# lrm2017/Fastest_Image_Pattern_Matching

Hardware: AMD Instinct MI355X
Metric: template matches/sec + ms/search, 4024×3036 src ±180°; HBM GB/s vs roofline (higher is better)
Workload: dtype u8

## Files before the change

### fastest_image_pattern_matching_amd/_lib.py

```python
from __future__ import annotations

import ctypes as C
import os
import subprocess

_HERE = os.path.dirname(os.path.abspath(__file__))
LIB_PATH = os.path.join(_HERE, "lib", "libfpm_hip.so")
CSRC = os.path.join(_HERE, "csrc")

FPM_OK = 0
FPM_E_INVALID_ARG = -1
FPM_E_NOT_LEARNED = -2
FPM_E_SIZE = -3
FPM_E_DEVICE = -4
FPM_E_CAPACITY = -5
FPM_E_INTERNAL = -6

(FMT_GRAY8, FMT_BGR8, FMT_RGB8, FMT_BGRA8, FMT_RGBA8, FMT_BGR8_PLANAR, FMT_RGB8_PLANAR) = range(7)
FMT_COUNT = 7

(K_PYR, K_TOP_WARP, K_TOP_NCC, K_TOP_NMS, K_CAND_INIT, K_ROI_TABLES, K_ROI_WARP, K_ROI_CORR, K_ROI_EVAL, K_ROI_SMALL,
 K_CAND_STEP, K_TOP_MAP, K_NOT, K_PATCH, K_COMPARE, K_LEARN) = range(16)
KERNEL_NAMES = ["pyr_down", "top_warp", "top_ncc", "top_nms", "cand_init", "roi_tables", "roi_warp", "roi_corr",
                "roi_eval", "roi_small", "cand_step", "top_map", "bitwise_not", "patch_warp", "patch_compare"]
# ... 138 lines not shown
    _fields_ = [("x", C.c_int32), ("y", C.c_int32), ("score", C.c_float)]


PEAKS_STATS_CALL, PEAKS_STATS_JOB = 8, 4
PEAKS_RAN_BLOCKS, PEAKS_RAN_NMS, PEAKS_RAN_FAST, PEAKS_RAN_GREEDY = 1, 2, 4, 8
TOP_MAPS_STATS = 8
TOP_FUSED_STATS = 10
TOP_FORM_EXACT16, TOP_FORM_EXACT14, TOP_FORM_SMALL, TOP_FORM_LARGE = 0, 1, 2, 3

_P = C.c_void_p
_U8P = C.POINTER(C.c_uint8)
SIGNATURES = {
    "fpm_params_default": (None, [C.POINTER(Params)]),
    "fpm_abi_version": (C.c_int, []),
    "fpm_create": (C.c_int, [C.c_int, C.POINTER(_P)]),
    "fpm_destroy": (C.c_int, [_P]),
    "fpm_last_error": (C.c_char_p, [_P]),
    "fpm_set_params": (C.c_int, [_P, C.POINTER(Params)]),
    "fpm_get_params": (C.c_int, [_P, C.POINTER(Params)]),
    "fpm_learn": (C.c_int, [_P, _U8P, C.c_int32, C.c_int32, C.c_size_t]),
    "fpm_clear_pattern": (C.c_int, [_P]),
    "fpm_is_learned": (C.c_int, [_P]),
    "fpm_match": (C.c_int, [_P, _U8P, C.c_int32, C.c_int32, C.c_size_t, C.POINTER(Result), C.c_int32,
                            C.POINTER(C.c_int32), C.POINTER(C.c_double)]),
    "fpm_stage_sources": (C.c_int, [_P, C.POINTER(_U8P), C.c_int32, C.c_int32, C.c_int32, C.c_size_t]),
    "fpm_stage_sources_device": (C.c_int, [_P, C.POINTER(_P), C.c_int32, C.c_int32, C.c_int32, C.c_size_t, C.c_size_t,
                                           C.c_int32, _P]),
    "fpm_match_device": (C.c_int, [_P, _P, C.c_int32, C.c_int32, C.c_size_t, C.c_size_t, C.c_int32, _P,
                                   C.POINTER(Result), C.c_int32, C.POINTER(C.c_int32), C.POINTER(C.c_double)]),
    "fpm_match_staged": (C.c_int, [_P, C.POINTER(Result), C.c_int32, C.POINTER(C.c_int32)]),
    "fpm_match_staged_launch": (C.c_int, [_P]),
    "fpm_match_staged_finish": (C.c_int, [_P, C.POINTER(Result), C.c_int32, C.POINTER(C.c_int32)]),
    "fpm_op_pyr_down": (C.c_int, [_P, _U8P, C.c_int32, C.c_int32, C.c_size_t, _U8P, C.c_size_t]),
    "fpm_op_pyr_down2": (C.c_int, [_P, _U8P, C.c_int32, C.c_int32, C.c_size_t, _U8P, C.c_size_t, _U8P, C.c_size_t,
                                   C.c_int32, C.c_int32]),
    "fpm_op_bitwise_not": (C.c_int, [_P, _U8P, C.c_int32, C.c_int32, C.c_size_t, _U8P, C.c_size_t]),
    "fpm_op_to_gray": (C.c_int, [_P, _P, C.c_int32, C.c_int32, C.c_size_t, C.c_size_t, C.c_int32, C.c_int32, _U8P,
                                 C.c_size_t]),
    "fpm_op_warp_affine": (C.c_int, [_P, _U8P, C.c_int32, C.c_int32, C.c_size_t, C.POINTER(C.c_double), _U8P,
                                     C.c_int32, C.c_int32, C.c_size_t, C.c_int32]),
    "fpm_op_ncc_map": (C.c_int, [_P, _U8P, C.c_int32, C.c_int32, C.c_size_t, C.c_int32, C.c_int32,
                                 C.POINTER(C.c_float)]),
    "fpm_op_refine": (C.c_int, [_P, C.POINTER(_U8P), C.c_int32, C.c_int32, C.c_int32, C.c_size_t, C.c_int32,
                                C.POINTER(C.c_float), C.POINTER(C.c_double), C.c_int32, C.c_int32, C.c_int32, C.c_int32,
                                C.POINTER(RoiRecord), _U8P, C.POINTER(C.c_int32)]),
    "fpm_op_peaks": (C.c_int, [_P, C.POINTER(C.POINTER(C.c_float)), C.POINTER(C.c_int32), C.POINTER(C.c_int32),
                               C.c_int32, C.c_int32, C.c_int32, C.c_int32, C.c_int32, C.c_int32, C.c_double, C.c_double,
                               C.c_int32, C.c_int32, C.c_uint32, C.POINTER(Peak), C.POINTER(C.c_int32),
                               C.POINTER(C.c_int32)]),
    "fpm_op_top_maps": (C.c_int, [_P, C.c_int32, C.c_double, C.POINTER(C.c_int32), C.POINTER(C.c_int32),
                                  C.POINTER(C.c_int64), C.POINTER(C.c_int32), C.POINTER(C.c_int32), C.c_int32,
                                  C.POINTER(C.c_float), C.c_int64, C.POINTER(C.c_int32), C.POINTER(C.c_int32),
                                  C.POINTER(C.c_float), C.c_int64, C.POINTER(C.c_int32)]),
    "fpm_op_top_fused": (C.c_int, [_P, C.POINTER(C.c_int32), C.POINTER(C.c_int32), C.POINTER(C.c_int64),
                                   C.POINTER(C.c_int32), C.POINTER(C.c_int32), C.c_int32, C.POINTER(C.c_float),
                                   C.c_int64, C.POINTER(Peak), C.POINTER(C.c_int32), C.POINTER(Peak),
                                   C.POINTER(C.c_int32), C.c_int64, C.POINTER(C.c_int32)]),
    "fpm_op_overlap_filter": (C.c_int, [_P, C.POINTER(C.c_float), C.POINTER(C.c_double), C.c_int32, C.c_double,
                                        C.c_int32, C.POINTER(C.c_int32), C.POINTER(C.c_int32), C.POINTER(C.c_int32)]),
    "fpm_template_info": (C.c_int, [_P, C.POINTER(C.c_int32), C.POINTER(C.c_int32)]),
    "fpm_template_level": (C.c_int, [_P, C.c_int32, C.POINTER(C.c_int32), C.POINTER(C.c_int32),
                                     C.POINTER(C.c_double), C.POINTER(C.c_double), C.POINTER(C.c_double),
                                     C.POINTER(C.c_int32), _U8P, C.c_size_t]),
    "fpm_set_angle_shard": (C.c_int, [_P, C.c_int32, C.c_int32]),
    "fpm_get_angle_shard": (C.c_int, [_P, C.POINTER(C.c_int32), C.POINTER(C.c_int32)]),
    "fpm_last_candidates": (C.c_int, [_P, C.c_int32, C.POINTER(Candidate), C.c_int32, C.POINTER(C.c_int32)]),
# ... 130 lines not shown
```

### fastest_image_pattern_matching_amd/csrc/fpm_engine.hip

```cpp
#include <hip/hip_runtime.h>

#include <algorithm>
#include <array>
#include <cfloat>
#include <chrono>
#include <cmath>
#include <cstddef>
#include <cstdio>
#include <cstdlib>
#include <cstring>
#include <new>
#include <random>
#include <string>
#include <vector>

#include "../../include/fpm.h"
#include "fpm_host.h"
#include "fpm_kernels.h"
#include "fpm_model.h"

using namespace fpm;

namespace {

// ... 3734 lines not shown
    if (!ctx->learned) return FPM_E_NOT_LEARNED;
    if (level < 0 || level >= (int)ctx->tmpl.size()) return FPM_E_INVALID_ARG;
    const TmplLevel& t = ctx->tmpl[level];
    *w = t.w; *h = t.h; *mean = t.mean; *norm = t.norm; *inv_area = t.inv_area; *result_equal1 = t.equal1 ? 1 : 0;
    if (pixels && t.px.empty()) {
        std::vector<uint8_t> px((size_t)t.w * t.h);
        if (hipSetDevice(ctx->device) != hipSuccess ||
            hipMemcpy2D(px.data(), t.w, ctx->d_tmpl.as<uint8_t>() + t.off, t.pitch, t.w, t.h, hipMemcpyDeviceToHost) != hipSuccess)
            return FPM_E_DEVICE;
        t.px = std::move(px);
    }
    if (pixels)
        for (int y = 0; y < t.h; ++y) std::memcpy(pixels + (size_t)y * stride, t.px.data() + (size_t)y * t.w, (size_t)t.w);
    return FPM_OK;
}

int fpm_op_pyr_down(fpm_ctx* ctx, const uint8_t* src, int32_t w, int32_t h, size_t ss, uint8_t* dst, size_t ds) {
    if (!ctx) return FPM_E_INVALID_ARG;
    if (!src || !dst || w <= 0 || h <= 0 || ss < (size_t)w) { ctx->err = "bad image"; return FPM_E_INVALID_ARG; }
    const int dw = (w + 1) / 2, dh = (h + 1) / 2;
    if (ds < (size_t)dw) { ctx->err = "bad dst stride"; return FPM_E_INVALID_ARG; }
    HIP_TRY(hipSetDevice(ctx->device));
    const int sp = round_up(w + 4, 64), dp = round_up(dw + 4, 64);
    HIP_TRY(ctx->d_op_a.ensure((size_t)sp * (h + 1)));
    HIP_TRY(ctx->d_op_b.ensure((size_t)dp * (dh + 1)));
    HIP_TRY(hipMemcpy2DAsync(ctx->d_op_a.p, sp, src, ss, w, h, hipMemcpyHostToDevice, ctx->stream));
    launch_pyr_down(ctx->d_op_a.as<uint8_t>(), w, h, sp, 0, ctx->d_op_b.as<uint8_t>(), dw, dh, dp, 0, 1, ctx->stream, 3);
    HIP_TRY(hipGetLastError());
    HIP_TRY(hipMemcpy2DAsync(dst, ds, ctx->d_op_b.p, dp, dw, dh, hipMemcpyDeviceToHost, ctx->stream));
    HIP_TRY(hipStreamSynchronize(ctx->stream));
    return FPM_OK;
}

int fpm_op_bitwise_not(fpm_ctx* ctx, const uint8_t* src, int32_t w, int32_t h, size_t ss, uint8_t* dst, size_t ds) {
    if (!ctx) return FPM_E_INVALID_ARG;
    if (!src || !dst || w <= 0 || h <= 0 || ss < (size_t)w) { ctx->err = "bad image"; return FPM_E_INVALID_ARG; }
    if (ds < (size_t)w) { ctx->err = "bad dst stride"; return FPM_E_INVALID_ARG; }
    HIP_TRY(hipSetDevice(ctx->device));
    const SrcLevel lv = level_layout(w, h);
    HIP_TRY(ctx->d_op_a.ensure(lv.img_bytes));
    HIP_TRY(hipMemcpy2DAsync(ctx->d_op_a.p, lv.pitch, src, ss, w, h, hipMemcpyHostToDevice, ctx->stream));
    {
        ProfScope ps(ctx, FPM_K_NOT, 2 * (int64_t)w * h);
        if (!launch_bitwise_not(ctx->d_op_a.as<uint8_t>(), w, h, lv.pitch, lv.img_bytes, 1, ctx->stream)) {
            ctx->err = "level layout: rows not 16-byte aligned";
            return FPM_E_INTERNAL;
        }
    }
    HIP_TRY(hipGetLastError());
    HIP_TRY(hipMemcpy2DAsync(dst, ds, ctx->d_op_a.p, lv.pitch, w, h, hipMemcpyDeviceToHost, ctx->stream));
    HIP_TRY(hipStreamSynchronize(ctx->stream));
    prof_collect(ctx);
    return FPM_OK;
}

int fpm_op_to_gray(fpm_ctx* ctx, const void* src, int32_t w, int32_t h, size_t ss, size_t plane_stride, int32_t format,
                   int32_t invert, uint8_t* dst, size_t ds) {
    if (!ctx) return FPM_E_INVALID_ARG;
    if (!src || !dst) { ctx->err = "bad image"; return FPM_E_INVALID_ARG; }
    const int rc = check_image_desc(ctx, 1, w, h, ss, plane_stride, format);
    if (rc != FPM_OK) return rc;
    if (ds < (size_t)w) { ctx->err = "bad dst stride"; return FPM_E_INVALID_ARG; }
    HIP_TRY(hipSetDevice(ctx->device));
    const size_t extent = image_extent(w, h, ss, plane_stride, format);
    const size_t mis = (uintptr_t)src & 15;
    const SrcLevel lv = level_layout(w, h);
// ... 640 lines not shown
```

### fastest_image_pattern_matching_amd/csrc/fpm_kernels.h

```cpp
#pragma once
#include <hip/hip_runtime.h>
#include <stdint.h>

#include "fpm_geom.h"

namespace fpm {

struct WarpJob {
    const uint8_t* src;
    uint8_t* dst;
    int32_t sw, sh, sp;
    int32_t dw, dh, dp;
    int32_t border;
    int32_t pad;
    double M[6];
};

struct NccJob {
    const uint8_t* img;
    const uint8_t* tmpl;
    float* out;
    int32_t iw, ih, ip;
    int32_t tw, th, tp;
    int32_t ow, oh;
// ... 100 lines not shown
    int32_t step;
    int32_t mark_reached0;
    int32_t* live_out;
    int32_t* live_out_count;
    double thr;
    const RoiRecord* prev_rec;
    const AngleNode* prev_nodes;
    double prev_thr;
    int32_t prev_W, prev_H;
    CandState* state_out;
    int32_t* nt_tab;
    const AngleNode* nt_nodes;
    int32_t nt_tabw, nt_tabh, nt_tw, nt_th, nt_W, nt_H;
    uint64_t* stamps;
};


struct PackArgs {
    const int32_t* counts; int32_t J;
    const Peak* peaks; int32_t C;
    int32_t cap;
    const int32_t* livecnt; int32_t nlive;
    const int32_t* live0;
    const int32_t* live0_count;
    const CandState* state;
    const RoiRecord* rec;
    int32_t n3;
    char* host;
    size_t o_counts, o_peaks, o_live, o_live0, o_state0, o_rec0;
};

void launch_pyr_down(const uint8_t* src, int sw, int sh, int sp, size_t s_img, uint8_t* dst, int dw, int dh,
                     int dp, size_t d_img, int nimg, hipStream_t st, int seg_chunks = 0, int32_t* zero = nullptr,
                     int nzero = 0);
void launch_pyr_down2(const uint8_t* src, int sw, int sh, int sp, size_t s_img, uint8_t* bdst, int bw, int bh, int bp,
                      size_t b_img, uint8_t* cdst, int cw, int ch, int cp, size_t c_img, int nimg, hipStream_t st,
                      int seg_chunks = 0, int32_t* zero = nullptr, int nzero = 0, int chunk_rows = 0);
bool launch_bitwise_not(uint8_t* img, int w, int h, int pitch, size_t img_bytes, int nimg, hipStream_t st);
bool launch_stage_gray(const uint8_t* const* d_imgs, int nimg, int w, int h, size_t stride, size_t plane_stride,
                       int format, bool aligned, uint8_t* dst, int pitch, size_t img_bytes, bool invert,
                       hipStream_t st);
int stage_gray_bpp(int format);
void launch_warp(const WarpJob* jobs, int njobs, int max_pixels, hipStream_t st, int32_t* zero = nullptr,
                 int nzero = 0);
struct PatchJob {
    double M[6];
    int64_t out_off;
    int32_t src;
    int32_t pad;
};
struct PatchArgs {
    const PatchJob* jobs;
    int32_t njobs;
    const uint8_t* level0;
    size_t img_stride;
    int32_t sw, sh, sp;
    uint8_t* out;
    size_t row_stride;
    int32_t pw, ph;
    int32_t dword;
    int32_t tiles_x, tiles_y;
};
bool launch_patch_warp(PatchArgs a, hipStream_t st);
enum { kCmpSumI, kCmpSumII, kCmpSumT, kCmpSumTT, kCmpSumIT, kCmpSumAbs, kCmpNOver, kCmpMaxAbs, kCmpX0, kCmpY0, kCmpX1,
       kCmpY1, kCompareFields };
struct CompareAcc {
    uint64_t s[6];
// ... 234 lines not shown
```

### fastest_image_pattern_matching_amd/csrc/fpm_kernels.hip

```cpp
#include <float.h>
#include <stdio.h>
#include <stdlib.h>
#include <limits.h>

#include <map>
#include <mutex>
#include <type_traits>
#include <utility>

#include "../../include/fpm.h"
#include "fpm_kernels.h"
#include "fpm_model.h"
#include "fpm_rrect.h"

static void ensure_lds_attr(const void* fn, size_t bytes) {
    if (bytes <= 65536) return;
    int dev = 0;
    (void)hipGetDevice(&dev);
    static std::mutex mu;
    static std::map<std::pair<int, const void*>, size_t> done;
    std::lock_guard<std::mutex> lock(mu);
    size_t& cur = done[std::make_pair(dev, fn)];
    if (bytes <= cur) return;
    (void)hipFuncSetAttribute(fn, hipFuncAttributeMaxDynamicSharedMemorySize, (int)bytes);
// ... 164 lines not shown
        const uint32_t h2 = __builtin_amdgcn_udot4(PD_K, __builtin_amdgcn_alignbyte(w2, w1, 2), 0, false) + ((w2 >> 16) & 0xff);
        const uint32_t h3 = __builtin_amdgcn_udot4(PD_K, w2, 0, false) + (w3 & 0xff);
        uint2 o;
        o.x = h0 | (h1 << 16);
        o.y = h2 | (h3 << 16);
        *(uint2*)&hs[r][4 * g] = o;
    }
    __syncthreads();
    if (ABL == 3) { if (hs[tid & 63][tid >> 1] == 0x5a5a && tid == 999) dst[0] = 1; return; }
#pragma unroll
    for (int k = 0; k < PD_OH * (PD_OW / 4) / 256; ++k) {
        const int i = tid + 256 * k;
        const int orow = i / (PD_OW / 4), g = i - orow * (PD_OW / 4);
        const int oy = oy0 + orow, ox = ox0 + 4 * g;
        if (oy >= dh || ox >= dw) continue;
        uint32_t acc[4] = {128, 128, 128, 128};
        const int kw[5] = {1, 4, 6, 4, 1};
#pragma unroll
        for (int t = 0; t < 5; ++t) {
            const uint2 q = *(const uint2*)&hs[2 * orow + t][4 * g];
            acc[0] += kw[t] * (q.x & 0xffff); acc[1] += kw[t] * (q.x >> 16);
            acc[2] += kw[t] * (q.y & 0xffff); acc[3] += kw[t] * (q.y >> 16);
        }
        uint8_t* d = dst + (size_t)oy * dp + ox;
        if (ox + 4 <= dw) {
            *(uint32_t*)d = (acc[0] >> 8) | ((acc[1] >> 8) << 8) | ((acc[2] >> 8) << 16) | ((acc[3] >> 8) << 24);
        } else {
            for (int j = 0; j < dw - ox; ++j) d[j] = (uint8_t)(acc[j] >> 8);
        }
    }
}

typedef unsigned short fpm_u16x2 __attribute__((ext_vector_type(2)));

template <int OH>
__global__ __launch_bounds__(256) void k_pyr_down_s(const uint8_t* __restrict__ src0, int sw, int sh, int sp,
                                                    size_t s_img, uint8_t* __restrict__ dst0, int dw, int dh,
                                                    int dp, size_t d_img, int nimg, int32_t* zero, int nzero) {
    constexpr int IH = 2 * OH + 4;
    constexpr int PS_NL = (IH * (PD_IW / 16) + 255) / 256;
    __shared__ __attribute__((aligned(16))) uint8_t tin[IH][PD_IW];
    if (blockIdx.x == 0)
        for (int i = threadIdx.x; i < nzero; i += 256) zero[i] = 0;
    __shared__ __attribute__((aligned(16))) uint16_t hs[IH][PD_OW];
    const int gx = (dw + PD_OW - 1) / PD_OW, chunks = (dh + OH - 1) / OH;
    const long U = (long)gx * chunks * nimg;
    const int w = xcd_remap(blockIdx.x, gridDim.x);
    long u = U * w / gridDim.x;
    const long u_end = U * (w + 1) / gridDim.x;
    const int tid = threadIdx.x;
    while (u < u_end) {
        const long strip = u / chunks;
        const int c0 = (int)(u - strip * chunks);
        const int run = (int)min(u_end - u, (long)(chunks - c0));
        u += run;
        const int bx = (int)(strip % gx), bz = (int)(strip / gx);
        const uint8_t* src = src0 + (size_t)bz * s_img;
        uint8_t* dst = dst0 + (size_t)bz * d_img;
        const int ox0 = bx * PD_OW;
        const int oy_begin = c0 * OH, oy_end = min(dh, (c0 + run) * OH);
        __syncthreads();
        const int ix0 = 2 * ox0 - 16;
        constexpr int Q = PD_IW / 16;
        auto srow = [&](int y) {
            y = y < 0 ? -y : y;
            y = y >= sh ? 2 * sh - 2 - y : y;
            return y < 0 ? 0 : (y >= sh ? sh - 1 : y);
        };
        uint4 v[PS_NL];
        auto issue = [&](int iy, int nrows) {
#pragma unroll
            for (int k = 0; k < PS_NL; ++k) {
                const int i = tid + 256 * k;
                const int r = i / Q, c = i - r * Q;
                const int x = ix0 + 16 * c;
                v[k] = make_uint4(0, 0, 0, 0);
                if (r < nrows && x >= 0 && x + 16 <= sp) v[k] = *(const uint4*)(src + (size_t)srow(iy + r) * sp + x);
            }
        };
        auto commit = [&](int roff, int nrows) {
#pragma unroll
            for (int k = 0; k < PS_NL; ++k) {
                const int i = tid + 256 * k;
                const int r = i / Q, c = i - r * Q;
                if (r < nrows) *(uint4*)&tin[roff + r][16 * c] = v[k];
            }
        };
        const int xlo = 2 * ox0 - 2, xhi = min(2 * (ox0 + PD_OW - 1) + 2, 2 * (dw - 1) + 2);
        const bool edge = xlo < 0 || xhi >= sw;
        issue(2 * oy_begin - 2, IH);
        for (int oyc = oy_begin; oyc < oy_end; oyc += OH) {
            const bool first = oyc == oy_begin;
            const int roff = first ? 0 : 4, nrows = first ? IH : 2 * OH;
            const int iy = 2 * oyc - 2 + roff;
            commit(roff, nrows);
            if (edge) {
                __syncthreads();
                for (int i = tid; i < nrows * 4; i += 256) {
                    const int r = i >> 2, k = i & 3;
                    const int x = k < 2 ? xlo + k : xhi - (k - 2);
                    if ((x < 0 && k < 2) || (x >= sw && k >= 2))
                        tin[roff + r][x - ix0] = src[(size_t)srow(iy + r) * sp + reflect101(x, sw)];
                }
            }
            __syncthreads();
            if (oyc + OH < oy_end) issue(2 * oyc + 2 * OH + 2, 2 * OH);
            const int nh = nrows * (PD_OW / 4);
            for (int i = tid; i < nh; i += 256) {
                const int r = roff + i / (PD_OW / 4), g = i % (PD_OW / 4);
                const uint32_t* w = (const uint32_t*)&tin[r][8 * g + 12];
                const uint32_t w0 = w[0], w1 = w[1], w2 = w[2], w3 = w[3];
                const uint32_t h0 = __builtin_amdgcn_udot4(PD_K, __builtin_amdgcn_alignbyte(w1, w0, 2), (w1 >> 16) & 0xff, false);
                const uint32_t h1 = __builtin_amdgcn_udot4(PD_K, w1, w2 & 0xff, false);
                const uint32_t h2 = __builtin_amdgcn_udot4(PD_K, __builtin_amdgcn_alignbyte(w2, w1, 2), (w2 >> 16) & 0xff, false);
                const uint32_t h3 = __builtin_amdgcn_udot4(PD_K, w2, w3 & 0xff, false);
                uint2 o;
                o.x = h0 | (h1 << 16);
                o.y = h2 | (h3 << 16);
                *(uint2*)&hs[r][4 * g] = o;
            }
            __syncthreads();
#pragma unroll
            for (int k = 0; k < OH * (PD_OW / 4) / 256; ++k) {
                const int i = tid + 256 * k;
                const int orow = i / (PD_OW / 4), g = i - orow * (PD_OW / 4);
                const int oy = oyc + orow, ox = ox0 + 4 * g;
                if (oy >= oy_end || ox >= dw) continue;
                fpm_u16x2 a01 = {128, 128}, a23 = {128, 128};
                constexpr unsigned short kw[5] = {1, 4, 6, 4, 1};
#pragma unroll
                for (int tt = 0; tt < 5; ++tt) {
                    const uint2 q = *(const uint2*)&hs[2 * orow + tt][4 * g];
                    a01 += __builtin_bit_cast(fpm_u16x2, q.x) * kw[tt];
                    a23 += __builtin_bit_cast(fpm_u16x2, q.y) * kw[tt];
                }
                const uint32_t packed = __builtin_amdgcn_perm(__builtin_bit_cast(uint32_t, a23),
                                                              __builtin_bit_cast(uint32_t, a01), 0x07050301u);
                uint8_t* d = dst + (size_t)oy * dp + ox;
                if (ox + 4 <= dw) {
                    *(uint32_t*)d = packed;
                } else {
                    for (int j = 0; j < dw - ox; ++j) d[j] = (uint8_t)(packed >> (8 * j));
                }
            }
            __syncthreads();
            ((uint32_t*)hs[tid >> 6])[tid & 63] = ((uint32_t*)hs[2 * OH + (tid >> 6)])[tid & 63];
            __syncthreads();
        }
    }
}

static const int kPyrWGs = [] {
    const char* e = getenv("FPM_PYR_WGS");
    return e && atoi(e) > 0 ? atoi(e) : 4096;
}();
static const int kPyrOH = [] {
    const char* e = getenv("FPM_PYR_OH");
    return e && atoi(e) == 16 ? 16 : 32;
}();
void launch_pyr_down(const uint8_t* src, int sw, int sh, int sp, size_t s_img, uint8_t* dst, int dw, int dh,
                     int dp, size_t d_img, int nimg, hipStream_t st, int seg_chunks, int32_t* zero, int nzero) {
    if (dw <= 0 || dh <= 0 || nimg <= 0) return;
    const int oh = kPyrOH;
    const int gx = (dw + PD_OW - 1) / PD_OW, chunks = (dh + oh - 1) / oh;
    const long units = (long)gx * chunks * nimg;
    const long g = seg_chunks > 0 ? (units + seg_chunks - 1) / seg_chunks : std::min(units, (long)kPyrWGs);
    if (oh == 16)
        hipLaunchKernelGGL(k_pyr_down_s<16>, dim3((unsigned)g), dim3(256), 0, st, src, sw, sh, sp, s_img, dst, dw, dh,
                           dp, d_img, nimg, zero, nzero);
    else
        hipLaunchKernelGGL(k_pyr_down_s<32>, dim3((unsigned)g), dim3(256), 0, st, src, sw, sh, sp, s_img, dst, dw, dh,
                           dp, d_img, nimg, zero, nzero);
}

constexpr int PD2_OWC = 64;
constexpr int PD2_OWB = 2 * PD2_OWC + 8;
constexpr int PD2_GB = PD2_OWB / 4;
constexpr int PD2_BP = 136;
template <int PD2_OHB>
__global__ __launch_bounds__(256) void k_pyr_down2(const uint8_t* __restrict__ src0, int sw, int sh, int sp,
                                                   size_t s_img, uint8_t* __restrict__ b0, int bw, int bh, int bpp,
                                                   size_t b_img, uint8_t* __restrict__ c0, int cw, int ch, int cpp,
                                                   size_t c_img, int nimg, int32_t* zero, int nzero) {
    constexpr int PD2_IH = 2 * (PD2_OHB + 4) + 4, PD2_RING = PD2_OHB + 6;
    __shared__ __attribute__((aligned(16))) uint8_t tin[PD2_IH][PD_IW];
    __shared__ __attribute__((aligned(16))) uint16_t hs[PD2_IH][PD2_BP];
    __shared__ __attribute__((aligned(16))) uint8_t ring[PD2_RING][PD2_BP];
    __shared__ __attribute__((aligned(16))) uint16_t hc[PD2_RING][PD2_OWC];
    if (blockIdx.x == 0)
        for (int i = threadIdx.x; i < nzero; i += 256) zero[i] = 0;
    const int gx = (cw + PD2_OWC - 1) / PD2_OWC, chunks = (bh + PD2_OHB - 1) / PD2_OHB;
    const long U = (long)gx * chunks * nimg;
    const int w = xcd_remap(blockIdx.x, gridDim.x);
    long u = U * w / gridDim.x;
    const long u_end = U * (w + 1) / gridDim.x;
    const int tid = threadIdx.x;
    constexpr int Q = PD_IW / 16;
    constexpr int NL = (PD2_IH * Q + 255) / 256;
    constexpr unsigned short kw[5] = {1, 4, 6, 4, 1};
    auto srow = [&](int y) {
        y = y < 0 ? -y : y;
        y = y >= sh ? 2 * sh - 2 - y : y;
        return y < 0 ? 0 : (y >= sh ? sh - 1 : y);
    };
    while (u < u_end) {
// ... 5380 lines not shown
```

### fastest_image_pattern_matching_amd/matcher.py

```python
from __future__ import annotations

import ctypes as C
import os
from dataclasses import dataclass
from typing import List, Sequence, Tuple

import numpy as np

from . import _lib as L


@dataclass
class SingleTargetMatch:

    ptLT: Tuple[float, float]
    ptRT: Tuple[float, float]
    ptRB: Tuple[float, float]
    ptLB: Tuple[float, float]
    ptCenter: Tuple[float, float]
    dMatchedAngle: float
    dMatchScore: float

    @staticmethod
    def from_c(r: "L.Result") -> "SingleTargetMatch":
# ... 1204 lines not shown
                                             edges.ctypes.data_as(C.POINTER(L.Edge)),
                                             prof.ctypes.data_as(C.POINTER(C.c_int32)) if profiles else None, stride,
                                             n.value, C.byref(n))
            if rc != L.FPM_OK:
                self._patch_fail(rc, "last_calipers")
        return (summary, edges, prof) if profiles else (summary, edges)

    def calipers_at(self, src_index, lts, angles, cals, cap: int = 8, profiles: bool = False):
        idx, lt, ang = patch_poses(src_index, lts, angles)
        arr = _calipers(cals)
        summary, edges, prof, stride = self._caliper_buffers(len(idx), arr, cap, profiles)
        rc = self._lib.fpm_calipers_at(self._ctx, idx.ctypes.data_as(C.POINTER(C.c_int32)),
                                       lt.ctypes.data_as(C.POINTER(C.c_float)), ang.ctypes.data_as(C.POINTER(C.c_double)),
                                       len(idx), arr.ctypes.data_as(C.POINTER(L.Caliper)), len(arr), int(cap),
                                       summary.ctypes.data_as(C.POINTER(L.CaliperSummary)),
                                       edges.ctypes.data_as(C.POINTER(L.Edge)),
                                       prof.ctypes.data_as(C.POINTER(C.c_int32)) if profiles else None, stride)
        if rc != L.FPM_OK:
            self._patch_fail(rc, "calipers_at")
        return (summary, edges, prof) if profiles else (summary, edges)

    def caliper_profile(self):
        ms, n, b = C.c_double(), C.c_int64(), C.c_int64()
        if self._lib.fpm_caliper_profile(self._ctx, C.byref(ms), C.byref(n), C.byref(b)) != L.FPM_OK:
            raise ValueError("fpm_caliper_profile failed")
        return ms.value, n.value, b.value

    def pyr_down(self, img) -> np.ndarray:
        g = _gray(img)
        h, w = g.shape
        out = np.zeros(((h + 1) // 2, (w + 1) // 2), np.uint8)
        rc = self._check(self._lib.fpm_op_pyr_down(self._ctx, L.u8ptr(g), w, h, g.strides[0], L.u8ptr(out),
                                                   out.strides[0]), "pyr_down")
        if rc != L.FPM_OK:
            raise ValueError(self.last_error())
        return out

    def bitwise_not(self, img) -> np.ndarray:
        a = np.asarray(img)
        strided = a.ndim == 2 and a.dtype == np.uint8 and a.shape[1] > 0 and a.strides[1] == 1 and a.strides[0] >= a.shape[1]
        g = a if strided else _gray(a)
        h, w = g.shape
        out = np.zeros((h, w), np.uint8)
        rc = self._check(self._lib.fpm_op_bitwise_not(self._ctx, L.u8ptr(g), w, h, g.strides[0], L.u8ptr(out),
                                                      out.strides[0]), "bitwise_not")
        if rc != L.FPM_OK:
            raise ValueError(self.last_error())
        return out

    def to_gray(self, img, channel_order: str = "bgr", layout=None, invert: bool = False, dst=None) -> np.ndarray:
        a = np.asarray(img)
        if a.dtype != np.uint8:
            raise TypeError(f"expected a uint8 array, got {a.dtype}")
        kind, h, w, ch, row, plane = device_layout(a.shape, a.strides, layout)
        fmt = device_format(kind, ch, channel_order)
        out = np.zeros((h, w), np.uint8) if dst is None else dst
        if out.dtype != np.uint8 or out.shape != (h, w) or (w > 1 and out.strides[1] != 1) or (h > 1 and out.strides[0] < w):
            raise ValueError(f"dst must be a ({h}, {w}) uint8 array with unit pixel stride")
        rc = self._check(self._lib.fpm_op_to_gray(self._ctx, a.ctypes.data, w, h, row, plane, fmt, 1 if invert else 0,
                                                  L.u8ptr(out), out.strides[0] if h > 1 else max(out.strides[0], w)),
                         "to_gray")
        if rc != L.FPM_OK:
            raise ValueError(self.last_error())
        return out

    def pyr_down2(self, img, seg_chunks: int = 0, chunk_rows: int = 0):
# ... 222 lines not shown
```

### include/fpm.h

```cpp
#ifndef FPM_H_
#define FPM_H_

#include <stddef.h>
#include <stdint.h>

#ifdef __cplusplus
extern "C" {
#endif

#define FPM_ABI_VERSION 11

#define FPM_OK 0
#define FPM_E_INVALID_ARG (-1)
#define FPM_E_NOT_LEARNED (-2)
#define FPM_E_SIZE (-3)
#define FPM_E_DEVICE (-4)
#define FPM_E_CAPACITY (-5)
#define FPM_E_INTERNAL (-6)

#define FPM_SEMANTICS_QT 0
#define FPM_SEMANTICS_MFC 1

typedef struct fpm_params {
    int32_t max_pos;
// ... 231 lines not shown
int fpm_caliper_pose(float lt_x, float lt_y, double angle, const fpm_caliper* cal, float* ltk_x, float* ltk_y,
                     double* angle_k);
int fpm_caliper_edges_host(const int32_t* profile, const fpm_caliper* cal, int32_t cap_per_caliper, fpm_edge_raw* out,
                           int32_t* n_edges, int32_t* flags);
int fpm_caliper_derive(const fpm_caliper* cal, float ltk_x, float ltk_y, double angle_k, const fpm_edge_raw* raw,
                       int32_t n, fpm_edge* out);
int fpm_calipers_at(fpm_ctx* ctx, const int32_t* src_index, const float* lt, const double* angles, int32_t n_poses,
                    const fpm_caliper* cals, int32_t n_cals, int32_t cap_per_caliper, fpm_caliper_summary* summary,
                    fpm_edge* edges, int32_t* profiles, int32_t profile_stride);
int fpm_last_calipers(fpm_ctx* ctx, int32_t source, const fpm_caliper* cals, int32_t n_cals, int32_t cap_per_caliper,
                      fpm_caliper_summary* summary, fpm_edge* edges, int32_t* profiles, int32_t profile_stride,
                      int32_t cap , int32_t* n);
int fpm_caliper_profile(const fpm_ctx* ctx, double* ms, int64_t* launches, int64_t* bytes);

typedef struct fpm_candidate {
    double top_score;
    double x, y;
    double score;
    double angle;
    int32_t angle_index;
    int32_t peak_rank;
    int32_t source;
    int32_t kept;
} fpm_candidate;

int fpm_set_angle_shard(fpm_ctx* ctx, int32_t shard, int32_t shards);
int fpm_get_angle_shard(const fpm_ctx* ctx, int32_t* shard, int32_t* shards);
int fpm_last_candidates(const fpm_ctx* ctx, int32_t source, fpm_candidate* out, int32_t cap, int32_t* n);
int fpm_merge_candidates(const fpm_params* p, int32_t tmpl_w, int32_t tmpl_h, const fpm_candidate* cand, int32_t n,
                         fpm_result* out, int32_t cap, int32_t* n_results);

int fpm_op_pyr_down(fpm_ctx* ctx, const uint8_t* src, int32_t w, int32_t h, size_t src_stride,
                    uint8_t* dst, size_t dst_stride);
int fpm_op_pyr_down2(fpm_ctx* ctx, const uint8_t* src, int32_t w, int32_t h, size_t src_stride,
                     uint8_t* dst1, size_t dst1_stride, uint8_t* dst2, size_t dst2_stride, int32_t seg_chunks,
                     int32_t chunk_rows);
int fpm_op_bitwise_not(fpm_ctx* ctx, const uint8_t* src, int32_t w, int32_t h, size_t src_stride,
                       uint8_t* dst, size_t dst_stride);
int fpm_op_to_gray(fpm_ctx* ctx, const void* src, int32_t w, int32_t h, size_t src_stride, size_t plane_stride,
                   int32_t format, int32_t invert, uint8_t* dst, size_t dst_stride);
int fpm_op_warp_affine(fpm_ctx* ctx, const uint8_t* src, int32_t w, int32_t h, size_t src_stride,
                       const double m[6], uint8_t* dst, int32_t dw, int32_t dh, size_t dst_stride,
                       int32_t border);
int fpm_op_ncc_map(fpm_ctx* ctx, const uint8_t* src, int32_t w, int32_t h, size_t src_stride,
                   int32_t layer, int32_t fold, float* out);
int fpm_op_overlap_filter(fpm_ctx* ctx, const float* corners, const double* scores, int32_t n, double max_overlap,
                          int32_t mode, int32_t* keep, int32_t* n_keep, int32_t* stats);
typedef struct fpm_roi_record {
    float score;
    int32_t mx, my;
    int32_t on_border;
    float vec[9];
} fpm_roi_record;
int fpm_op_refine(fpm_ctx* ctx, const uint8_t* const* levels, int32_t count, int32_t w, int32_t h, size_t stride,
                  int32_t layer, const float* lt, const double* angles, int32_t n, int32_t n3, int32_t fold,
                  int32_t round_rois, fpm_roi_record* rec, uint8_t* roi_pixels, int32_t* pixels_written);
typedef struct fpm_peak {
    int32_t x, y;
    float score;
} fpm_peak;
#define FPM_PEAKS_MAX_PIXELS (1 << 26)
#define FPM_PEAKS_MAX_SLOTS (1 << 24)
#define FPM_PEAKS_STATS_CALL 8
#define FPM_PEAKS_STATS_JOB 4
int fpm_op_peaks(fpm_ctx* ctx, const float* const* maps, const int32_t* mw, const int32_t* mh, int32_t n_maps,
                 int32_t tw, int32_t th, int32_t cap, int32_t by_block, int32_t mfc, double thr, double overlap,
// ... 51 lines not shown
```

Baseline: 37310.

## Pipeline pyr_down source rows via direct global-to-LDS loads with multi-stage buffering

Rewrites the single-pass pyramid-down kernel so source row tiles are fetched with global_load_lds_dwordx4 straight into shared memory, using an NS-stage ring of buffers and explicit vmcnt waits instead of register staging and __syncthreads. The horizontal pass is reorganised so each thread handles fixed rows, and the vertical pass now produces two output rows per thread. The 4-row halo is carried between chunks in alternating buffers rather than copied. A new op entry point exposes chunk_rows and seg_chunks for testing. The inline asm that manipulates M0 and the hand-counted waits add fragility and the risk of subtle races.

```diff
diff --git a/fastest_image_pattern_matching_amd/_lib.py b/fastest_image_pattern_matching_amd/_lib.py
--- a/fastest_image_pattern_matching_amd/_lib.py
+++ b/fastest_image_pattern_matching_amd/_lib.py
@@ -194,6 +194,7 @@
     "fpm_match_staged_launch": (C.c_int, [_P]),
     "fpm_match_staged_finish": (C.c_int, [_P, C.POINTER(Result), C.c_int32, C.POINTER(C.c_int32)]),
     "fpm_op_pyr_down": (C.c_int, [_P, _U8P, C.c_int32, C.c_int32, C.c_size_t, _U8P, C.c_size_t]),
+    "fpm_op_pyr_down_runs": (C.c_int, [_P, _U8P, C.c_int32, C.c_int32, C.c_size_t, _U8P, C.c_size_t, C.c_int32, C.c_int32]),
     "fpm_op_pyr_down2": (C.c_int, [_P, _U8P, C.c_int32, C.c_int32, C.c_size_t, _U8P, C.c_size_t, _U8P, C.c_size_t,
                                    C.c_int32, C.c_int32]),
     "fpm_op_bitwise_not": (C.c_int, [_P, _U8P, C.c_int32, C.c_int32, C.c_size_t, _U8P, C.c_size_t]),
diff --git a/fastest_image_pattern_matching_amd/csrc/fpm_engine.hip b/fastest_image_pattern_matching_amd/csrc/fpm_engine.hip
--- a/fastest_image_pattern_matching_amd/csrc/fpm_engine.hip
+++ b/fastest_image_pattern_matching_amd/csrc/fpm_engine.hip
@@ -3790,6 +3790,28 @@
     return FPM_OK;
 }
 
+int fpm_op_pyr_down_runs(fpm_ctx* ctx, const uint8_t* src, int32_t w, int32_t h, size_t ss, uint8_t* dst, size_t ds,
+                         int32_t seg_chunks, int32_t chunk_rows) {
+    if (!ctx) return FPM_E_INVALID_ARG;
+    if (!src || !dst || w <= 0 || h <= 0 || ss < (size_t)w || seg_chunks < 0 || (chunk_rows != 16 && chunk_rows != 32)) {
+        ctx->err = "bad image";
+        return FPM_E_INVALID_ARG;
+    }
+    const int dw = (w + 1) / 2, dh = (h + 1) / 2;
+    if (ds < (size_t)dw) { ctx->err = "bad dst stride"; return FPM_E_INVALID_ARG; }
+    HIP_TRY(hipSetDevice(ctx->device));
+    const int sp = round_up(w + 4, 64), dp = round_up(dw + 4, 64);
+    HIP_TRY(ctx->d_op_a.ensure((size_t)sp * (h + 1)));
+    HIP_TRY(ctx->d_op_b.ensure((size_t)dp * (dh + 1)));
+    HIP_TRY(hipMemcpy2DAsync(ctx->d_op_a.p, sp, src, ss, w, h, hipMemcpyHostToDevice, ctx->stream));
+    launch_pyr_down(ctx->d_op_a.as<uint8_t>(), w, h, sp, 0, ctx->d_op_b.as<uint8_t>(), dw, dh, dp, 0, 1, ctx->stream,
+                    seg_chunks, nullptr, 0, chunk_rows);
+    HIP_TRY(hipGetLastError());
+    HIP_TRY(hipMemcpy2DAsync(dst, ds, ctx->d_op_b.p, dp, dw, dh, hipMemcpyDeviceToHost, ctx->stream));
+    HIP_TRY(hipStreamSynchronize(ctx->stream));
+    return FPM_OK;
+}
+
 int fpm_op_bitwise_not(fpm_ctx* ctx, const uint8_t* src, int32_t w, int32_t h, size_t ss, uint8_t* dst, size_t ds) {
     if (!ctx) return FPM_E_INVALID_ARG;
     if (!src || !dst || w <= 0 || h <= 0 || ss < (size_t)w) { ctx->err = "bad image"; return FPM_E_INVALID_ARG; }
diff --git a/fastest_image_pattern_matching_amd/csrc/fpm_kernels.h b/fastest_image_pattern_matching_amd/csrc/fpm_kernels.h
--- a/fastest_image_pattern_matching_amd/csrc/fpm_kernels.h
+++ b/fastest_image_pattern_matching_amd/csrc/fpm_kernels.h
@@ -156,7 +156,7 @@
 
 void launch_pyr_down(const uint8_t* src, int sw, int sh, int sp, size_t s_img, uint8_t* dst, int dw, int dh,
                      int dp, size_t d_img, int nimg, hipStream_t st, int seg_chunks = 0, int32_t* zero = nullptr,
-                     int nzero = 0);
+                     int nzero = 0, int chunk_rows = 0);
 void launch_pyr_down2(const uint8_t* src, int sw, int sh, int sp, size_t s_img, uint8_t* bdst, int bw, int bh, int bp,
                       size_t b_img, uint8_t* cdst, int cw, int ch, int cp, size_t c_img, int nimg, hipStream_t st,
                       int seg_chunks = 0, int32_t* zero = nullptr, int nzero = 0, int chunk_rows = 0);
diff --git a/fastest_image_pattern_matching_amd/csrc/fpm_kernels.hip b/fastest_image_pattern_matching_amd/csrc/fpm_kernels.hip
--- a/fastest_image_pattern_matching_amd/csrc/fpm_kernels.hip
+++ b/fastest_image_pattern_matching_amd/csrc/fpm_kernels.hip
@@ -220,23 +220,69 @@
 }
 
 typedef unsigned short fpm_u16x2 __attribute__((ext_vector_type(2)));
-
-template <int OH>
+typedef __attribute__((address_space(3))) const uint8_t fpm_pd_lds_u8;
+
+__device__ __forceinline__ void pd_wait_vm(int n) {
+    switch (n) {
+    case 0: asm volatile("s_waitcnt vmcnt(0)" ::: "memory"); break;
+    case 1: asm volatile("s_waitcnt vmcnt(1)" ::: "memory"); break;
+    case 2: asm volatile("s_waitcnt vmcnt(2)" ::: "memory"); break;
+    case 3: asm volatile("s_waitcnt vmcnt(3)" ::: "memory"); break;
+    case 4: asm volatile("s_waitcnt vmcnt(4)" ::: "memory"); break;
+    case 5: asm volatile("s_waitcnt vmcnt(5)" ::: "memory"); break;
+    case 6: asm volatile("s_waitcnt vmcnt(6)" ::: "memory"); break;
+    case 7: asm volatile("s_waitcnt vmcnt(7)" ::: "memory"); break;
+    default: asm volatile("s_waitcnt vmcnt(8)" ::: "memory"); break;
+    }
+}
+__device__ __forceinline__ void pd_barrier() { asm volatile("s_waitcnt lgkmcnt(0)\n\ts_barrier" ::: "memory"); }
+__device__ __forceinline__ void pd_dma(const uint8_t* base, uint32_t off, uint32_t lds) {
+    uint32_t keep;
+    asm volatile("s_mov_b32 %0, m0\n\ts_mov_b32 m0, %3\n\ts_nop 0\n\tglobal_load_lds_dwordx4 %1, %2\n\ts_mov_b32 m0, %0"
+                 : "=&s"(keep) : "v"(off), "s"(base), "s"(lds) : "memory");
+}
+__device__ __forceinline__ void pd_dma_p(const uint8_t* p, uint32_t lds) {
+    uint32_t keep;
+    asm volatile("s_mov_b32 %0, m0\n\ts_mov_b32 m0, %2\n\ts_nop 0\n\tglobal_load_lds_dwordx4 %1, off\n\ts_mov_b32 m0, %0"
+                 : "=&s"(keep) : "v"(p), "s"(lds) : "memory");
+}
+
+template <int OH, int NS>
 __global__ __launch_bounds__(256) void k_pyr_down_s(const uint8_t* __restrict__ src0, int sw, int sh, int sp,
                                                     size_t s_img, uint8_t* __restrict__ dst0, int dw, int dh,
                                                     int dp, size_t d_img, int nimg, int32_t* zero, int nzero) {
-    constexpr int IH = 2 * OH + 4;
-    constexpr int PS_NL = (IH * (PD_IW / 16) + 255) / 256;
-    __shared__ __attribute__((aligned(16))) uint8_t tin[IH][PD_IW];
+    constexpr int NR = 2 * OH;
+    constexpr int Q = PD_IW / 16;
+    constexpr int NP = NR * Q;
+    constexpr int NL = (NP + 255) / 256;
+    constexpr int SB = NR * PD_IW;
+    constexpr int HEAD = NS * SB;
+    constexpr int HSA = HEAD + 4 * PD_IW;
+    constexpr int HSM = HSA + 4 * 256;
+    constexpr int HSB = HSM + NR * 256;
+    constexpr int ST = OH / 8;
+    __shared__ __attribute__((aligned(16))) uint8_t smem[HSB + 4 * 256];
     if (blockIdx.x == 0)
         for (int i = threadIdx.x; i < nzero; i += 256) zero[i] = 0;
-    __shared__ __attribute__((aligned(16))) uint16_t hs[IH][PD_OW];
     const int gx = (dw + PD_OW - 1) / PD_OW, chunks = (dh + OH - 1) / OH;
     const long U = (long)gx * chunks * nimg;
     const int w = xcd_remap(blockIdx.x, gridDim.x);
     long u = U * w / gridDim.x;
     const long u_end = U * (w + 1) / gridDim.x;
-    const int tid = threadIdx.x;
+    const int tid = threadIdx.x, wv = __builtin_amdgcn_readfirstlane(tid >> 6);
+    const int hr = tid >> 5, hg = tid & 31;
+    const int nlw = (NP - 64 * wv + 255) / 256;
+    const uint32_t wlds = __builtin_amdgcn_readfirstlane((uint32_t)(size_t)(fpm_pd_lds_u8*)smem) + 1024u * (uint32_t)wv;
+    int rck[NL], xck[NL];
+#pragma unroll
+    for (int k = 0; k < NL; ++k) {
+        const int i = tid + 256 * k, r = i / Q, c = i - r * Q;
+        rck[k] = r * sp + 16 * c;
+        xck[k] = 16 * c;
+    }
+    const uint8_t* const tl = smem + hr * PD_IW + 8 * hg + 12;
+    uint8_t* const hl = smem + HSM + hr * 256 + 8 * hg;
+    const uint8_t* const vl = smem + HSA + 4 * hr * 256 + 8 * hg;
     while (u < u_end) {
         const long strip = u / chunks;
         const int c0 = (int)(u - strip * chunks);
@@ -247,56 +293,83 @@
         uint8_t* dst = dst0 + (size_t)bz * d_img;
         const int ox0 = bx * PD_OW;
         const int oy_begin = c0 * OH, oy_end = min(dh, (c0 + run) * OH);
-        __syncthreads();
         const int ix0 = 2 * ox0 - 16;
-        constexpr int Q = PD_IW / 16;
         auto srow = [&](int y) {
             y = y < 0 ? -y : y;
             y = y >= sh ? 2 * sh - 2 - y : y;
             return y < 0 ? 0 : (y >= sh ? sh - 1 : y);
         };
-        uint4 v[PS_NL];
-        auto issue = [&](int iy, int nrows) {
-#pragma unroll
-            for (int k = 0; k < PS_NL; ++k) {
-                const int i = tid + 256 * k;
-                const int r = i / Q, c = i - r * Q;
-                const int x = ix0 + 16 * c;
-                v[k] = make_uint4(0, 0, 0, 0);
-                if (r < nrows && x >= 0 && x + 16 <= sp) v[k] = *(const uint4*)(src + (size_t)srow(iy + r) * sp + x);
-            }
-        };
-        auto commit = [&](int roff, int nrows) {
-#pragma unroll
-            for (int k = 0; k < PS_NL; ++k) {
-                const int i = tid + 256 * k;
-                const int r = i / Q, c = i - r * Q;
-                if (r < nrows) *(uint4*)&tin[roff + r][16 * c] = v[k];
+        uint32_t offk[NL];
+        bool okk[NL];
+#pragma unroll
+        for (int k = 0; k < NL; ++k) {
+            const int x = ix0 + xck[k];
+            okk[k] = x >= 0 && x + 16 <= sp;
+            offk[k] = okk[k] ? (uint32_t)(rck[k] + ix0) : 0u;
+        }
+        auto issue = [&](int m) {
+            const int iy = 2 * (oy_begin + m * OH) + 2;
+            const uint32_t lds = wlds + (uint32_t)((m % NS) * SB);
+            if (iy + NR <= sh) {
+                const uint8_t* rowp = src + (size_t)iy * sp;
+#pragma unroll
+                for (int k = 0; k < NL; ++k)
+                    if (k < nlw) {
+                        if (okk[k]) pd_dma(rowp, offk[k], lds + 4096u * k);
+                    }
+            } else {
+#pragma unroll
+                for (int k = 0; k < NL; ++k)
+                    if (k < nlw) {
+                        const int r = (tid + 256 * k) / Q;
+                        if (okk[k]) pd_dma_p(src + (size_t)srow(iy + r) * sp + (ix0 + xck[k]), lds + 4096u * k);
+                    }
             }
         };
         const int xlo = 2 * ox0 - 2, xhi = min(2 * (ox0 + PD_OW - 1) + 2, 2 * (dw - 1) + 2);
         const bool edge = xlo < 0 || xhi >= sw;
-        issue(2 * oy_begin - 2, IH);
-        for (int oyc = oy_begin; oyc < oy_end; oyc += OH) {
-            const bool first = oyc == oy_begin;
-            const int roff = first ? 0 : 4, nrows = first ? IH : 2 * OH;
-            const int iy = 2 * oyc - 2 + roff;
-            commit(roff, nrows);
+        auto patch = [&](uint8_t* rows, int nrows) {
+            for (int i = tid; i < nrows * 4; i += 256) {
+                const int r = i >> 2, k = i & 3;
+                const int x = k < 2 ? xlo + k : xhi - (k - 2);
+                if ((x < 0 && k < 2) || (x >= sw && k >= 2))
+                    rows[r * PD_IW + x - ix0] = rows[r * PD_IW + reflect101(x, sw) - ix0];
+            }
+        };
+        const bool strip_full = ox0 + PD_OW <= dw;
+        const int nch = (oy_end - oy_begin + OH - 1) / OH;
+        auto nst = [&](int m) { return m >= 0 && strip_full && oy_begin + (m + 1) * OH <= oy_end ? ST : 0; };
+        if (tid < 4 * Q) {
+            const int r = tid / Q, c = tid - r * Q, x = ix0 + 16 * c;
+            if (x >= 0 && x + 16 <= sp)
+                pd_dma_p(src + (size_t)srow(2 * oy_begin - 2 + r) * sp + x, wlds + (uint32_t)HEAD);
+        }
+        issue(0);
+#pragma unroll
+        for (int j = 1; j <= NS - 2; ++j)
+            if (j < nch) issue(j);
+        for (int n = 0; n < nch; ++n) {
+            const int oyc = oy_begin + n * OH;
+            const int stage = (n % NS) * SB;
+            int N = 0;
+            if (NS >= 2) {
+#pragma unroll
+                for (int j = 1; j <= NS - 2; ++j) N += n + j < nch ? nlw : 0;
+#pragma unroll
+                for (int m = 1; m <= NS - 1; ++m) N += nst(n - m);
+            } else {
+                N = nst(n - 1);
+            }
+            pd_wait_vm(N);
+            pd_barrier();
             if (edge) {
-                __syncthreads();
-                for (int i = tid; i < nrows * 4; i += 256) {
-                    const int r = i >> 2, k = i & 3;
-                    const int x = k < 2 ? xlo + k : xhi - (k - 2);
-                    if ((x < 0 && k < 2) || (x >= sw && k >= 2))
-                        tin[roff + r][x - ix0] = src[(size_t)srow(iy + r) * sp + reflect101(x, sw)];
-                }
-            }
-            __syncthreads();
-            if (oyc + OH < oy_end) issue(2 * oyc + 2 * OH + 2, 2 * OH);
-            const int nh = nrows * (PD_OW / 4);
-            for (int i = tid; i < nh; i += 256) {
-                const int r = roff + i / (PD_OW / 4), g = i % (PD_OW / 4);
-                const uint32_t* w = (const uint32_t*)&tin[r][8 * g + 12];
+                if (n == 0) patch(smem + HEAD, 4);
+                patch(smem + stage, NR);
+                pd_barrier();
+            }
+            if (NS >= 2 && n + NS - 1 < nch) issue(n + NS - 1);
+            auto hitem = [&](const uint8_t* tp) {
+                const uint32_t* w = (const uint32_t*)tp;
                 const uint32_t w0 = w[0], w1 = w[1], w2 = w[2], w3 = w[3];
                 const uint32_t h0 = __builtin_amdgcn_udot4(PD_K, __builtin_amdgcn_alignbyte(w1, w0, 2), (w1 >> 16) & 0xff, false);
                 const uint32_t h1 = __builtin_amdgcn_udot4(PD_K, w1, w2 & 0xff, false);
@@ -305,39 +378,62 @@
                 uint2 o;
                 o.x = h0 | (h1 << 16);
                 o.y = h2 | (h3 << 16);
-                *(uint2*)&hs[r][4 * g] = o;
-            }
-            __syncthreads();
-#pragma unroll
-            for (int k = 0; k < OH * (PD_OW / 4) / 256; ++k) {
-                const int i = tid + 256 * k;
-                const int orow = i / (PD_OW / 4), g = i - orow * (PD_OW / 4);
-                const int oy = oyc + orow, ox = ox0 + 4 * g;
-                if (oy >= oy_end || ox >= dw) continue;
-                fpm_u16x2 a01 = {128, 128}, a23 = {128, 128};
-                constexpr unsigned short kw[5] = {1, 4, 6, 4, 1};
-#pragma unroll
-                for (int tt = 0; tt < 5; ++tt) {
-                    const uint2 q = *(const uint2*)&hs[2 * orow + tt][4 * g];
-                    a01 += __builtin_bit_cast(fpm_u16x2, q.x) * kw[tt];
-                    a23 += __builtin_bit_cast(fpm_u16x2, q.y) * kw[tt];
-                }
+                return o;
+            };
+            uint8_t* const cnext = smem + ((n & 1) ? HSA : HSB) + (hr - 4) * 256 + 8 * hg;
+            if (n == 0 && tid < 128) *(uint2*)(smem + HSA + hr * 256 + 8 * hg) = hitem(smem + HEAD + hr * PD_IW + 8 * hg + 12);
+#pragma unroll
+            for (int j = 0; j < NR / 8; ++j) {
+                const uint2 o = hitem(tl + stage + j * 8 * PD_IW);
+                *(uint2*)(hl + j * 8 * 256) = o;
+                if (j == NR / 8 - 1 && wv >= 2) *(uint2*)cnext = o;
+            }
+            pd_barrier();
+            if (NS == 1 && n + 1 < nch) issue(n + 1);
+            const bool full = strip_full && oyc + OH <= oy_end;
+            const bool carry_b = wv == 0 && (n & 1);
+            const int ox = ox0 + 4 * hg;
+            auto put = [&](uint8_t* d, int oy, fpm_u16x2 a01, fpm_u16x2 a23) {
+                if (!full && (oy >= oy_end || ox >= dw)) return;
                 const uint32_t packed = __builtin_amdgcn_perm(__builtin_bit_cast(uint32_t, a23),
                                                               __builtin_bit_cast(uint32_t, a01), 0x07050301u);
-                uint8_t* d = dst + (size_t)oy * dp + ox;
-                if (ox + 4 <= dw) {
+                if (full || ox + 4 <= dw) {
                     *(uint32_t*)d = packed;
                 } else {
-                    for (int j = 0; j < dw - ox; ++j) d[j] = (uint8_t)(packed >> (8 * j));
-                }
-            }
-            __syncthreads();
-            ((uint32_t*)hs[tid >> 6])[tid & 63] = ((uint32_t*)hs[2 * OH + (tid >> 6)])[tid & 63];
-            __syncthreads();
-        }
-    }
-}
-
+                    d[0] = (uint8_t)packed;
+                    if (ox + 2 <= dw) d[1] = (uint8_t)(packed >> 8);
+                    if (ox + 3 <= dw) d[2] = (uint8_t)(packed >> 16);
+                }
+            };
+            constexpr unsigned short kw[5] = {1, 4, 6, 4, 1};
+            uint8_t* d = dst + (size_t)(oyc + 2 * hr) * dp + ox;
+#pragma unroll
+            for (int k = 0; k < OH / 16; ++k, d += (size_t)16 * dp) {
+                const int oy = oyc + 2 * (hr + 8 * k);
+                if (!full && (oy >= oy_end || ox >= dw)) continue;
+                uint2 q[7];
+#pragma unroll
+                for (int tt = 0; tt < 7; ++tt) {
+                    const uint8_t* hp = vl + (32 * k + tt) * 256;
+                    if (k == 0 && carry_b && 4 * hr + tt < 4) hp = smem + HSB + (4 * hr + tt) * 256 + 8 * hg;
+                    q[tt] = *(const uint2*)hp;
+                }
+                fpm_u16x2 a01 = {128, 128}, a23 = {128, 128}, b01 = {128, 128}, b23 = {128, 128};
+#pragma unroll
+                for (int tt = 0; tt < 5; ++tt) {
+                    a01 += __builtin_bit_cast(fpm_u16x2, q[tt].x) * kw[tt];
+                    a23 += __builtin_bit_cast(fpm_u16x2, q[tt].y) * kw[tt];
+                    b01 += __builtin_bit_cast(fpm_u16x2, q[tt + 2].x) * kw[tt];
+                    b23 += __builtin_bit_cast(fpm_u16x2, q[tt + 2].y) * kw[tt];
+                }
+                put(d, oy, a01, a23);
+                put(d + dp, oy + 1, b01, b23);
+            }
+        }
+    }
+}
+
+constexpr int kPyrStages16 = 3, kPyrStages32 = 1;
 static const int kPyrWGs = [] {
     const char* e = getenv("FPM_PYR_WGS");
     return e && atoi(e) > 0 ? atoi(e) : 4096;
@@ -347,18 +443,19 @@
     return e && atoi(e) == 16 ? 16 : 32;
 }();
 void launch_pyr_down(const uint8_t* src, int sw, int sh, int sp, size_t s_img, uint8_t* dst, int dw, int dh,
-                     int dp, size_t d_img, int nimg, hipStream_t st, int seg_chunks, int32_t* zero, int nzero) {
+                     int dp, size_t d_img, int nimg, hipStream_t st, int seg_chunks, int32_t* zero, int nzero,
+                     int chunk_rows) {
     if (dw <= 0 || dh <= 0 || nimg <= 0) return;
-    const int oh = kPyrOH;
+    const int oh = chunk_rows == 16 || chunk_rows == 32 ? chunk_rows : kPyrOH;
     const int gx = (dw + PD_OW - 1) / PD_OW, chunks = (dh + oh - 1) / oh;
     const long units = (long)gx * chunks * nimg;
     const long g = seg_chunks > 0 ? (units + seg_chunks - 1) / seg_chunks : std::min(units, (long)kPyrWGs);
     if (oh == 16)
-        hipLaunchKernelGGL(k_pyr_down_s<16>, dim3((unsigned)g), dim3(256), 0, st, src, sw, sh, sp, s_img, dst, dw, dh,
-                           dp, d_img, nimg, zero, nzero);
+        hipLaunchKernelGGL((k_pyr_down_s<16, kPyrStages16>), dim3((unsigned)g), dim3(256), 0, st, src, sw, sh, sp, s_img, dst, dw,
+                           dh, dp, d_img, nimg, zero, nzero);
     else
-        hipLaunchKernelGGL(k_pyr_down_s<32>, dim3((unsigned)g), dim3(256), 0, st, src, sw, sh, sp, s_img, dst, dw, dh,
-                           dp, d_img, nimg, zero, nzero);
+        hipLaunchKernelGGL((k_pyr_down_s<32, kPyrStages32>), dim3((unsigned)g), dim3(256), 0, st, src, sw, sh, sp, s_img, dst, dw,
+                           dh, dp, d_img, nimg, zero, nzero);
 }
 
 constexpr int PD2_OWC = 64;
diff --git a/fastest_image_pattern_matching_amd/matcher.py b/fastest_image_pattern_matching_amd/matcher.py
--- a/fastest_image_pattern_matching_amd/matcher.py
+++ b/fastest_image_pattern_matching_amd/matcher.py
@@ -1260,6 +1260,18 @@
         out = np.zeros(((h + 1) // 2, (w + 1) // 2), np.uint8)
         rc = self._check(self._lib.fpm_op_pyr_down(self._ctx, L.u8ptr(g), w, h, g.strides[0], L.u8ptr(out),
                                                    out.strides[0]), "pyr_down")
+        if rc != L.FPM_OK:
+            raise ValueError(self.last_error())
+        return out
+
+    def pyr_down_runs(self, img, seg_chunks: int = 0, chunk_rows: int = 32) -> np.ndarray:
+        a = np.asarray(img)
+        strided = a.ndim == 2 and a.dtype == np.uint8 and a.shape[1] > 0 and a.strides[1] == 1 and a.strides[0] >= a.shape[1]
+        g = a if strided else _gray(a)
+        h, w = g.shape
+        out = np.zeros(((h + 1) // 2, (w + 1) // 2), np.uint8)
+        rc = self._check(self._lib.fpm_op_pyr_down_runs(self._ctx, L.u8ptr(g), w, h, g.strides[0], L.u8ptr(out),
+                                                        out.strides[0], int(seg_chunks), int(chunk_rows)), "pyr_down_runs")
         if rc != L.FPM_OK:
             raise ValueError(self.last_error())
         return out
diff --git a/include/fpm.h b/include/fpm.h
--- a/include/fpm.h
+++ b/include/fpm.h
@@ -287,6 +287,8 @@
 
 int fpm_op_pyr_down(fpm_ctx* ctx, const uint8_t* src, int32_t w, int32_t h, size_t src_stride,
                     uint8_t* dst, size_t dst_stride);
+int fpm_op_pyr_down_runs(fpm_ctx* ctx, const uint8_t* src, int32_t w, int32_t h, size_t src_stride,
+                         uint8_t* dst, size_t dst_stride, int32_t seg_chunks, int32_t chunk_rows);
 int fpm_op_pyr_down2(fpm_ctx* ctx, const uint8_t* src, int32_t w, int32_t h, size_t src_stride,
                      uint8_t* dst1, size_t dst1_stride, uint8_t* dst2, size_t dst2_stride, int32_t seg_chunks,
                      int32_t chunk_rows);
```

After: 37630, median of 6. About the same (+0.8%).
